# Plachtaa/FAcodec

Measured on NVIDIA H100. Metric: audio_seconds_per_second, higher is better.
Workload: dtype f32 I/O and accumulation; every product is a 3-MMA split of fp32 operands: fp16 hi + 2^11-scaled fp16 lo (22 mantissa bits, register-promoted accumulation) upstream of the VQ, bf16 hi + bf16 lo (16 bits) downstream

## Files before the change

facodec_b200/csrc/conv_tc.cu:

```cuda
#include <cuda_bf16.h>
#include <cuda_fp16.h>

#include <cstring>
#include <mutex>
#include <type_traits>

#include "common.cuh"
#include "conv_tc_common.cuh"
#include "kernels.h"

namespace fac {

namespace {

using namespace tc;

enum Prec { P_TF32 = 0, P_BF16 = 1, P_F16S = 2, P_F16X2 = 3, P_NONE = -1 };

template <int P> struct PrecT {
    static constexpr int KG = P == P_TF32 ? 4 : 2;
    static constexpr int planes = P == P_F16S ? 1 : 2;
    static constexpr int ksteps = P == P_TF32 ? 2 : 1;
    static constexpr int kind = P == P_TF32 ? WG_TF32 : (P == P_BF16 ? WG_BF16 : WG_F16);
};
// ... 28 lines not shown
#pragma unroll
    for (int j = 0; j < NI / 8; ++j) {
        if (j > 0 && (8 * j) % GROUP == 0 && 8 * j >= tl.nw) break;
#pragma unroll
        for (int h = 0; h < 2; ++h) {
            const int row = tl.row0 + 16 * tl.warp + (tl.lane >> 2) + 8 * h;
            const int col = tl.col0 + 8 * j + 2 * (tl.lane & 3);
            f(row, col, acc[4 * j + 2 * h], acc[4 * j + 2 * h + 1]);
        }
    }
}

template <bool FAST>
__device__ __forceinline__ float act_out(int act, float v, float al, float ia) {
    if (act == ACT_SNAKE) return FAST ? fmaf(ia, sin2_mufu(al * v), v) : snake_fast(v, al, ia);
    if (act == ACT_TANH) return tanhf(v);
    if (act == ACT_MISH) return mish_f(v);
    return v;
}

template <int P1, int P2, bool TT>
constexpr bool groupable() { return P1 != P_F16S && P2 == P_NONE && !TT; }

template <int P1, int P2, bool PROMO, int NI, int MINB = 1, bool TT = false>
__global__ void __launch_bounds__(kThreads, groupable<P1, P2, TT>() && NI <= 128 ? 2 : MINB) conv_tc_kernel(TcConvParams p) {
    constexpr bool FUSED = P2 != P_NONE;
    constexpr bool GROUPABLE = groupable<P1, P2, TT>();
    static_assert(!TT || (NI == 64 && !FUSED), "transposed tiles: <= 64 channels x 64 time steps per warpgroup");
    static_assert(NI % 16 == 0 && NI <= (PROMO || MINB == 2 ? 64 : (P1 == P_F16S ? 256 : 128)),
                  "accumulator registers: <= 64 / 128 columns (256 in the one-pass fp16 class at one CTA per SM)");
    constexpr bool F16X2 = P1 == P_F16X2;
    constexpr bool DEC = P1 == P_BF16 || P1 == P_F16S;
    using T1 = PrecT<P1>;
    extern __shared__ __align__(1024) uint8_t smem[];
    uint64_t* full = reinterpret_cast<uint64_t*>(smem);

    const int tid = threadIdx.x, wg = tid >> 7;
    const int BM = 64 * p.MT;
    const int N = p.N, NW = p.MT == 2 ? N : N / 2;
    Tile tl;
    tl.row0 = p.MT == 2 ? 64 * wg : 0;
    tl.col0 = p.MT == 2 ? 0 : wg * NW;
    tl.nw = NW;
    tl.warp = (tid >> 5) & 3;
    tl.lane = tid & 31;
    const int t0 = blockIdx.x * BM, ntile = blockIdx.y, b = blockIdx.z;
    const int Kr = p.Kr, dil = p.dil, Rpad = p.Rpad, nchunk = p.nchunk, S = p.stagesB;
    const int G = GROUPABLE ? p.group : 1;
    const int R = BM + (Kr - 1) * dil;
    const int nstep1 = G == 4 ? nchunk >> 2 : (G == 2 ? nchunk >> 1 : nchunk);
    const uint32_t a_plane = (uint32_t)G * T1::KG * Rpad * 16, a_bytes = a_plane * T1::planes;
    uint8_t* abuf = smem + kSmemHdr;
    float4* master = reinterpret_cast<float4*>(abuf + 2 * (size_t)a_bytes);
    uint8_t* wbuf = abuf + 2 * (size_t)a_bytes + master_bytes(PROMO, nchunk, p.promote_every, NI);
    uint8_t* a2buf = wbuf + (size_t)S * p.b_slot;
    const uint32_t w_unit1 = (uint32_t)Kr * T1::planes * T1::KG * N * 16;
    const uint32_t w_unit2 = FUSED ? (uint32_t)prec_planes(P2) * prec_kg(P2) * N * 16 : 0;
    const int units = nstep1 + (FUSED ? p.nchunk2 : 0);

    if (tid == 0) {
        for (int i = 0; i < S; ++i) mbar_init(&full[i], 1);
        fence_mbar_init();
    }
    __syncthreads();
    auto issue_w = [&](int u) {
        uint64_t* bar = &full[u % S];
        uint8_t* dst = wbuf + (size_t)(u % S) * p.b_slot;
        const uint8_t* src;
        uint32_t bytes;
        if (u < nstep1) {
            src = reinterpret_cast<const uint8_t*>(p.wblob) + ((size_t)ntile * nchunk + (size_t)u * G) * w_unit1;
            bytes = G * w_unit1;
        } else { src = reinterpret_cast<const uint8_t*>(p.wblob2) + (size_t)(u - nstep1) * w_unit2; bytes = w_unit2; }
        mbar_arrive_expect_tx(bar, bytes);
        bulk_g2s(dst, src, bytes, bar);
    };
    if (tid == 0)
        for (int u = 0; u < S - 1 && u < units; ++u) issue_w(u);

    const PadMap pm = PadMap::lane(p.lane_len, b, p.Tin, p.pad_left_s, p.pad_right_s, p.reflect);
    const float* __restrict__ xb = p.x + (size_t)b * p.x_bstride;
    auto produce = [&](int s) {
        uint8_t* ahi = abuf + (size_t)(s & 1) * a_bytes;
        auto run = [&](auto grouped) {
            constexpr bool GR = decltype(grouped)::value;
            const int c = GR ? s * G : s;
            if constexpr (P1 == P_TF32) produce_chunk<kThreads, GR, false>(p, pm, xb, c, G, t0, R, Rpad, ahi, ahi + a_plane, tid);
            else if constexpr (P1 == P_BF16) produce_chunk<kThreads, GR, true>(p, pm, xb, c, G, t0, R, Rpad, ahi, ahi + a_plane, tid);
            else if constexpr (P1 == P_F16S) produce_chunk<kThreads, GR, true, 4, false, false, true>(p, pm, xb, c, G, t0, R, Rpad, ahi, ahi, tid);
            else produce_chunk<kThreads, GR, false, 4, false, true>(p, pm, xb, c, G, t0, R, Rpad, ahi, ahi + a_plane, tid);
        };
        if constexpr (GROUPABLE) {
            if (G > 1) run(std::true_type());
            else run(std::false_type());
        } else {
            run(std::false_type());
        }
        fence_proxy_async();
    };
    produce(0);

    float acc[NI / 2];
    float crs[F16X2 ? NI / 2 : 1];
    zero_acc<NI>(acc);
    if constexpr (F16X2) zero_acc<NI>(crs);
    const uint32_t a_lbo = (uint32_t)Rpad * 16, b_lbo = (uint32_t)N * 16;
    const uint32_t abase = smem_u32(abuf), wbase = smem_u32(wbuf), a2base = smem_u32(a2buf);
    const int BM2 = BM;
// ... 20 lines not shown
        }
    };

#pragma unroll 1
    for (int u = 0; u < units; ++u) {
        __syncthreads();
        if (tid == 0 && u + S - 1 < units) issue_w(u + S - 1);
        mbar_wait(&full[u % S], (uint32_t)(u / S) & 1u);
        const uint32_t wslot = wbase + (uint32_t)(u % S) * p.b_slot;
        wg_fence();
        if (u < nstep1) {
            const uint32_t a0 = abase + (uint32_t)(u & 1) * a_bytes + (uint32_t)tl.row0 * 16;
            const uint32_t b0 = wslot + (uint32_t)tl.col0 * 16;
            auto mma_tap = [&](uint32_t ahi, uint32_t bhi) {
                const uint32_t alo = ahi + a_plane, blo = bhi + T1::KG * b_lbo;
                if constexpr (TT) {
                    mma_pass<P1, NI>(acc, bhi, b_lbo, ahi, a_lbo);
                    mma_pass<P1, NI>(crs, bhi, b_lbo, alo, a_lbo);
                    mma_pass<P1, NI>(crs, blo, b_lbo, ahi, a_lbo);
                } else if constexpr (P1 == P_F16S) {
                    mma_pass<P1, NI>(acc, ahi, a_lbo, bhi, b_lbo);
                } else if constexpr (F16X2) {
                    mma_pass<P1, NI>(acc, ahi, a_lbo, bhi, b_lbo);
                    mma_pass<P1, NI>(crs, ahi, a_lbo, blo, b_lbo);
                    mma_pass<P1, NI>(crs, alo, a_lbo, bhi, b_lbo);
                } else {
                    mma_pass<P1, NI>(acc, ahi, a_lbo, bhi, b_lbo);
                    mma_pass<P1, NI>(acc, ahi, a_lbo, blo, b_lbo);
                    mma_pass<P1, NI>(acc, alo, a_lbo, bhi, b_lbo);
                }
            };
            if constexpr (GROUPABLE) {
                uint32_t ac = a0, bc = b0, ahi = a0, bhi = b0;
#pragma unroll 1
                for (int i = 0, tap = 0; i < G * Kr; ++i) {
                    mma_tap(ahi, bhi);
                    if (++tap < Kr) { ahi += (uint32_t)dil * 16; bhi += T1::planes * T1::KG * b_lbo; }
                    else { tap = 0; ac += T1::KG * a_lbo; bc += w_unit1; ahi = ac; bhi = bc; }
                }
            } else {
#pragma unroll 1
                for (int tap = 0; tap < Kr; ++tap)
                    mma_tap(a0 + (uint32_t)(tap * dil) * 16, b0 + (uint32_t)tap * T1::planes * T1::KG * b_lbo);
            }
            wg_commit();
            if (u + 1 < nstep1) produce(u + 1);
            wg_wait_all();
            const int done = (u + 1) * G;
            if (PROMO && (done % p.promote_every == 0 || done == nchunk)) promote(done <= p.promote_every, done == nchunk);
            if constexpr (FUSED) {
                if (u + 1 == nstep1) {
                    constexpr int KG2 = prec_kg(P2 < 0 ? 0 : P2);
                    const uint32_t a2_plane = (uint32_t)(p.nchunk2 * KG2) * BM2 * 16;
                    for_each_pair<NI, 32>(tl, acc, [&](int row, int col, float v0, float v1) {
                        const float2 bi = __ldg(reinterpret_cast<const float2*>(p.bias + col));
                        const float2 al = __ldg(reinterpret_cast<const float2*>(p.out_alpha + col));
                        const float2 ia = __ldg(reinterpret_cast<const float2*>(p.out_inv_alpha + col));
                        v0 = act_out<DEC>(ACT_SNAKE, v0 + bi.x, al.x, ia.x);
                        v1 = act_out<DEC>(ACT_SNAKE, v1 + bi.y, al.y, ia.y);
                        if constexpr (P2 == P_BF16) {
                            __nv_bfloat162 h = __floats2bfloat162_rn(v0, v1);
                            float2 hf = __bfloat1622float2(h);
                            __nv_bfloat162 l = __floats2bfloat162_rn(v0 - hf.x, v1 - hf.y);
                            const uint32_t off = ((uint32_t)(col >> 3) * BM2 + row) * 16 + (col & 7) * 2;
                            *reinterpret_cast<__nv_bfloat162*>(a2buf + off) = h;
                            *reinterpret_cast<__nv_bfloat162*>(a2buf + a2_plane + off) = l;
                        } else {
                            const float h0 = to_tf32(v0), h1 = to_tf32(v1);
                            const uint32_t off = ((uint32_t)(col >> 2) * BM2 + row) * 16 + (col & 3) * 4;
                            *reinterpret_cast<float2*>(a2buf + off) = make_float2(h0, h1);
                            *reinterpret_cast<float2*>(a2buf + a2_plane + off) = make_float2(to_tf32(v0 - h0), to_tf32(v1 - h1));
                        }
                    });
                    fence_proxy_async();
                    zero_acc<NI>(acc);
                }
            }
        } else if constexpr (FUSED) {
            constexpr int P2x = P2 < 0 ? 0 : P2;
            constexpr int KG2 = prec_kg(P2x);
            const int c2 = u - nstep1;
            const uint32_t a2_plane = (uint32_t)(p.nchunk2 * KG2) * BM2 * 16, a2_lbo = (uint32_t)BM2 * 16;
            const uint32_t ahi = a2base + ((uint32_t)(c2 * KG2) * BM2 + tl.row0) * 16, alo = ahi + a2_plane;
            const uint32_t bhi = wslot + (uint32_t)tl.col0 * 16, blo = bhi + KG2 * b_lbo;
            mma_pass<P2x, NI>(acc, ahi, a2_lbo, bhi, b_lbo);
            mma_pass<P2x, NI>(acc, ahi, a2_lbo, blo, b_lbo);
            mma_pass<P2x, NI>(acc, alo, a2_lbo, bhi, b_lbo);
            wg_commit();
            wg_wait_all();
        }
    }

    const float* __restrict__ bias = FUSED ? p.bias2 : p.bias;
    const int act = FUSED ? ACT_NONE : p.out_act;
    float* __restrict__ yb = p.y + (size_t)b * p.y_bstride + (size_t)ntile * N;
    const float* __restrict__ rb = p.res ? p.res + (size_t)b * p.y_bstride + (size_t)ntile * N : nullptr;
    const float* al_p = act == ACT_SNAKE ? p.out_alpha + (size_t)ntile * N : nullptr;
    const float* ia_p = act == ACT_SNAKE ? p.out_inv_alpha + (size_t)ntile * N : nullptr;
    const float* bi_p = bias ? bias + (size_t)ntile * N : nullptr;
    if constexpr (TT) {
        for_each_pair<NI>(tl, acc, [&](int r, int c, float v0, float v1) {
            if (r - tl.row0 >= NW) return;
            const int co = tl.col0 + (r - tl.row0), tf = tl.row0 + (c - tl.col0);
            const float bi = bi_p ? __ldg(bi_p + co) : 0.f;
            const float al = act == ACT_SNAKE ? __ldg(al_p + co) : 0.f, ia = act == ACT_SNAKE ? __ldg(ia_p + co) : 0.f;
            const float v[2] = {v0, v1};
#pragma unroll
            for (int e = 0; e < 2; ++e) {
                const int t = t0 + tf + e;
                if (t >= p.Tout) continue;
                float o = act_out<DEC>(act, v[e] + bi, al, ia);
                if (rb) o += rb[(size_t)t * p.ldy + co];
                yb[(size_t)t * p.ldy + co] = o;
            }
        });
        return;
    }
    for_each_pair<NI>(tl, acc, [&](int row, int col, float v0, float v1) {
        const int t = t0 + row;
        if (t >= p.Tout) return;
        if (bi_p) { const float2 bi = __ldg(reinterpret_cast<const float2*>(bi_p + col)); v0 += bi.x; v1 += bi.y; }
        if (act == ACT_SNAKE) {
            const float2 al = __ldg(reinterpret_cast<const float2*>(al_p + col));
            const float2 ia = __ldg(reinterpret_cast<const float2*>(ia_p + col));
            v0 = act_out<DEC>(ACT_SNAKE, v0, al.x, ia.x);
            v1 = act_out<DEC>(ACT_SNAKE, v1, al.y, ia.y);
        } else if (act != ACT_NONE) {
            v0 = act_out<DEC>(act, v0, 0.f, 0.f);
            v1 = act_out<DEC>(act, v1, 0.f, 0.f);
        }
        if (rb) { const float2 r = *reinterpret_cast<const float2*>(rb + (size_t)t * p.ldy + col); v0 += r.x; v1 += r.y; }
        *reinterpret_cast<float2*>(yb + (size_t)t * p.ldy + col) = make_float2(v0, v1);
    });
}

}

namespace {
constexpr size_t kSmemCap = 227 * 1024;
constexpr size_t kSmemCap2 = 113 * 1024;
int plan_prec(const TcConvParams& p) {
    return p.g1f16 ? P_F16S : (p.f16x2 ? P_F16X2 : (p.bf16 ? P_BF16 : P_TF32));
}
constexpr int f16s_wide_nw(bool fused) { return fused ? 192 : 256; }
}

bool tc_conv_plan(TcConvParams& p) {
    if ((p.Cin % 4) != 0 || ((p.Cin * p.vf) % kChunk) != 0 || (p.Cout % 16) != 0) return false;
    if (p.bf16 && p.promoted) return false;
    if (p.f16x2 && !p.promoted) return false;
    if (p.g1f16 && !p.bf16) return false;
    if (p.tt && !p.f16x2) return false;
    if (p.fused && (p.promoted || p.Cin != p.Cout || p.vf != 1 || p.Cout > 256)) return false;
    const int P1 = plan_prec(p), P2 = p.fused ? (p.bf16 ? P_BF16 : P_TF32) : P_NONE;
    p.nchunk = p.Cin * p.vf / kChunk;
    p.nchunk2 = p.fused ? p.Cout / kChunk : 0;
    p.promote_every = p.promoted ? (p.f16x2 ? (48 / p.Kr < 1 ? 1 : 48 / p.Kr) : (8 / p.Kr < 1 ? 1 : 8 / p.Kr)) : 1;
    const int nw_max = p.promoted ? 64 : 128;
    constexpr size_t kAReserve = 40 * 1024;
    int N = 0;
    for (int cand = p.fused ? p.Cout : 256; cand >= 16 && N == 0; cand -= 16) {
        const bool rows_split = cand <= nw_max, cols_split = (cand / 2) % 16 == 0 && cand / 2 <= nw_max;
        if (p.Cout % cand || !(rows_split || cols_split)) continue;
        size_t slot = (size_t)p.Kr * prec_planes(P1) * prec_kg(P1) * cand * 16, a2 = 0;
        if (P2 != P_NONE) a2 = (size_t)prec_planes(P2) * p.nchunk2 * prec_kg(P2) * 64 * 16;
        if (kSmemHdr + kAReserve + slot + a2 <= kSmemCap) N = cand;
        else if (p.fused) return false;
    }
    if (N == 0) return false;
    struct Layout { int Rpad; size_t slot, total; };
    auto layout = [&](int S, int MT, int G) {
        const int NW = MT == 2 ? N : N / 2, BM = 64 * MT;
        Layout l;
        const int v = G == 1 ? 2 : (P1 == P_TF32 ? 1 : 4 / G);
        l.Rpad = BM + (p.Kr - 1) * p.dil;
        while (l.Rpad % 8 != v) ++l.Rpad;
        const size_t a_bytes = (size_t)G * prec_planes(P1) * prec_kg(P1) * l.Rpad * 16;
        l.slot = (size_t)G * p.Kr * prec_planes(P1) * prec_kg(P1) * N * 16;
        size_t a2 = 0;
        if (P2 != P_NONE) {
            const size_t slot2 = (size_t)prec_planes(P2) * prec_kg(P2) * N * 16;
            if (slot2 > l.slot) l.slot = slot2;
            a2 = (size_t)prec_planes(P2) * p.nchunk2 * prec_kg(P2) * BM * 16;
        }
        const size_t master = master_bytes(p.promoted, p.nchunk, p.promote_every, p.tt ? 64 : NW);
        l.total = kSmemHdr + 2 * a_bytes + master + S * l.slot + a2 + (p.tt ? 64 * 16 : 0);
        return l;
    };
    auto group = [&](int S, int MT, size_t cap) {
        if (p.Kr > 3 || p.tt || p.fused || p.g1f16) return 1;
        for (int G = 4; G > 1; G /= 2)
            if (G <= p.max_group && p.nchunk % G == 0 && (!p.promoted || p.promote_every % G == 0) && layout(S, MT, G).total <= cap) return G;
        return 1;
    };
    const bool want2 = p.promoted ? !p.tt : (p.occ2_maxn > 0 && N <= p.occ2_maxn);
    for (int two = want2 ? 1 : 0; two >= 0; --two) {
        const size_t cap = two ? kSmemCap2 : kSmemCap;
        const int nwl = two ? 64 : nw_max;
        for (int S = 2; S >= 1; --S)
            for (int MT = 2; MT >= 1; --MT) {
                const int NW = MT == 2 ? N : N / 2;
                const bool wide = !two && P1 == P_F16S && NW == f16s_wide_nw(p.fused);
                if ((NW > nwl && !wide) || NW % 16) continue;
                if (wide && layout(2, 1, 1).total <= kSmemCap2) continue;
                const Layout l1 = layout(S, MT, 1);
                if (l1.total > cap) continue;
                const int G = group(S, MT, l1.total <= kSmemCap2 ? kSmemCap2 : cap);
                const Layout l = layout(S, MT, G);
                p.N = N; p.MT = MT; p.Rpad = l.Rpad; p.R2pad = 64 * MT; p.stagesB = S; p.b_slot = (int)l.slot;
                p.group = G;
                p.smem_bytes = l.total;
                p.occ2 = two;
                return true;
            }
    }
    return false;
}

size_t tc_blob_floats(const TcConvParams& p) {
    if (p.g1f16) return (size_t)(p.Cout / p.N) * p.nchunk * p.Kr * 2 * p.N * 4;
    return (size_t)(p.Cout / p.N) * p.nchunk * p.Kr * 2 * ((p.bf16 || p.f16x2) ? 2 : 4) * p.N * 4;
}

static inline uint16_t bf16_rn_host(float f) {
    uint32_t u;
    memcpy(&u, &f, 4);
    u += 0x7FFFu + ((u >> 16) & 1u);
    return (uint16_t)(u >> 16);
}

void tc_pack_blob(const TcConvParams& p, const float* wp, int ldw, float* blob) {
    const int Cw = p.Cin * p.vf;
    if (p.g1f16) {
        uint16_t* ob = reinterpret_cast<uint16_t*>(blob);
        size_t o16 = 0;
        for (int nt = 0; nt < p.Cout / p.N; ++nt)
            for (int c = 0; c < p.nchunk; ++c)
                for (int tap = 0; tap < p.Kr; ++tap)
                    for (int k8 = 0; k8 < 2; ++k8)
                        for (int n = 0; n < p.N; ++n)
                            for (int e = 0; e < 8; ++e) {
                                int kk = tap * Cw + c * tc::kChunk + k8 * 8 + e;
                                __half v = __float2half_rn(wp[(size_t)kk * ldw + nt * p.N + n]);
                                uint16_t bits;
                                memcpy(&bits, &v, 2);
                                ob[o16++] = bits;
                            }
        return;
    }
    if (p.f16x2) {
        uint16_t* ob = reinterpret_cast<uint16_t*>(blob);
        size_t o16 = 0;
        for (int nt = 0; nt < p.Cout / p.N; ++nt)
            for (int c = 0; c < p.nchunk; ++c)
                for (int tap = 0; tap < p.Kr; ++tap)
                    for (int hl = 0; hl < 2; ++hl)
// ... 51 lines not shown
                                lu = (lu + 0x1000u) & 0xFFFFE000u;
                                float lo_r;
                                memcpy(&lo_r, &lu, 4);
                                blob[o++] = hl == 0 ? hi : lo_r;
                            }
}

namespace {
template <int P1, int P2, bool PROMO, int NI, int MINB = 1, bool TT = false>
cudaError_t launch_one(const TcConvParams& p, dim3 grid, cudaStream_t st) {
    static bool done[64] = {};
    static std::mutex mu;
    int dev = 0;
    cudaError_t e = cudaGetDevice(&dev);
    if (e != cudaSuccess) return e;
    if (dev < 0 || dev >= 64) return cudaErrorInvalidDevice;
    {
        std::lock_guard<std::mutex> lk(mu);
        if (!done[dev]) {
            e = cudaFuncSetAttribute(conv_tc_kernel<P1, P2, PROMO, NI, MINB, TT>, cudaFuncAttributeMaxDynamicSharedMemorySize,
                                     (int)kSmemCap);
            if (e != cudaSuccess) return e;
            done[dev] = true;
        }
    }
    conv_tc_kernel<P1, P2, PROMO, NI, MINB, TT><<<grid, kThreads, p.smem_bytes, st>>>(p);
    return cudaGetLastError();
}
template <int P1, int P2, bool PROMO, int MINB = 1, int NI = (PROMO || MINB == 2 ? 64 : 128)>
cudaError_t launch_nw(const TcConvParams& p, dim3 grid, cudaStream_t st) {
    const int NW = p.MT == 2 ? p.N : p.N / 2;
    if (NW == NI) return launch_one<P1, P2, PROMO, NI, MINB>(p, grid, st);
    if constexpr (NI > 16) return launch_nw<P1, P2, PROMO, MINB, NI - 16>(p, grid, st);
    else return cudaErrorInvalidValue;
}
template <int P1, int P2>
cudaError_t launch_occ(const TcConvParams& p, dim3 grid, cudaStream_t st) {
    if (p.occ2) return launch_nw<P1, P2, false, 2>(p, grid, st);
    if constexpr (P1 == P_F16S) {
        constexpr int kWide = f16s_wide_nw(P2 != P_NONE);
        if ((p.MT == 2 ? p.N : p.N / 2) == kWide) return launch_one<P1, P2, false, kWide>(p, grid, st);
    }
    return launch_nw<P1, P2, false, 1>(p, grid, st);
}
}

cudaError_t launch_conv_tc(const TcConvParams& p, cudaStream_t st) {
    if (p.Tout <= 0 || p.B <= 0) return cudaSuccess;
    const int BM = 64 * p.MT;
    dim3 grid((p.Tout + BM - 1) / BM, p.Cout / p.N, p.B);
    if (grid.y > 65535 || grid.z > 65535) return cudaErrorInvalidValue;
    const int P1 = plan_prec(p);
    if (p.fused) {
        if (P1 == P_F16S) return launch_occ<P_F16S, P_BF16>(p, grid, st);
        if (P1 == P_BF16) return launch_occ<P_BF16, P_BF16>(p, grid, st);
        return launch_occ<P_TF32, P_TF32>(p, grid, st);
    }
    if (p.tt) return launch_one<P_F16X2, P_NONE, true, 64, 1, true>(p, grid, st);
    if (p.promoted)
        return P1 == P_F16X2 ? launch_nw<P_F16X2, P_NONE, true, 2>(p, grid, st) : launch_nw<P_TF32, P_NONE, true, 2>(p, grid, st);
    if (P1 == P_F16S) return launch_occ<P_F16S, P_NONE>(p, grid, st);
    if (P1 == P_BF16) return launch_occ<P_BF16, P_NONE>(p, grid, st);
    return launch_occ<P_TF32, P_NONE>(p, grid, st);
}

}
```

facodec_b200/csrc/engine.cu:

```cuda
#include <cmath>
#include <cstdio>
#include <cstdlib>
#include <cstring>
#include <algorithm>
#include <initializer_list>
#include <map>
#include <memory>
#include <string>
#include <type_traits>
#include <vector>

#include "../../include/facodec_b200.h"
#include "../../include/facodec_b200_debug.h"
#include "common.cuh"
#include "kernels.h"

using namespace fac;

namespace {

constexpr int HOP = 300;
constexpr int LATENT = 1024;
constexpr int N_FFT = 2048;
constexpr int WIN = 1200;
// ... 656 lines not shown
            tp.B = B; tp.Tin = Tin; tp.ldx = w.Cin;
            tp.PLr = o.pad_left / w.vf;
            tp.pad_left_s = o.pad_left; tp.pad_right_s = o.pad_right; tp.reflect = o.reflect; tp.lane_len = o.lane_len;
            tp.Tout = Tout; tp.ldy = w.Cout;
            tp.x_bstride = (size_t)Tin * w.Cin; tp.y_bstride = (size_t)Tout * w.Cout;
            double flops = 2.0 * B * Tout * (double)w.Cout * w.K * w.Cin;
            double bytes = 4.0 * ((double)B * Tin * w.Cin + (double)B * Tout * w.Cout * (o.res ? 2 : 1) + (double)w.K * w.Cin * w.Cout);
            char det[96];
            snprintf(det, sizeof det, "%s Cin%d Cout%d K%d d%d T%d", name, w.Cin, w.Cout, w.K, o.dil, Tout);
            c.begin(tp.promoted ? "conv_tcp" : "conv_tc", flops, bytes, det);
            c.check(launch_conv_tc(tp, c.st), name);
            c.end();
            return;
        }
    }
    ConvParams p;
    p.x = x; p.y = y;
    p.w = c.W(w.w);
    p.bias = o.no_bias ? nullptr : c.W(w.b);
    if (o.in_snake) { p.in_alpha = c.W(o.in_snake->a); p.in_inv_alpha = c.W(o.in_snake->ia); }
    p.out_act = o.act;
    if (o.out_snake) { p.out_act = ACT_SNAKE; p.out_alpha = c.W(o.out_snake->a); p.out_inv_alpha = c.W(o.out_snake->ia); }
    p.res = o.res; p.valid_len = o.valid_len; p.lane_len = o.lane_len;
    p.B = B; p.Tin = Tin; p.Cin = w.Cin; p.Tout = Tout; p.Cout = w.Cout;
    p.K = w.K; p.dil = o.dil; p.stride = o.stride;
    p.pad_left = o.pad_left; p.pad_right = o.pad_right; p.pad_reflect = o.reflect;
    p.ldw = w.ldw; p.ldy = o.ldy ? o.ldy : w.Cout; p.ldx = o.ldx ? o.ldx : w.Cin;
    p.y_transposed = o.transposed;
    p.x_bstride = (size_t)Tin * p.ldx;
    p.y_bstride = (size_t)Tout * p.ldy;
    double flops = 2.0 * B * Tout * (double)w.Cout * w.K * w.Cin;
    double bytes = 4.0 * ((double)B * Tin * w.Cin + (double)B * Tout * w.Cout * (o.res ? 2 : 1) + (double)w.K * w.Cin * w.Cout);
    char det[96];
    snprintf(det, sizeof det, "%s Cin%d Cout%d K%d d%d T%d", name, w.Cin, w.Cout, w.K, o.dil, Tout);
    c.begin("conv", flops, bytes, det);
    c.check(launch_conv(p, c.st), name);
    c.end();
}

int sconv(Ctx& c, const ConvW& w, const float* x, float* y, int B, int T, int dil, int stride, ConvOpts o,
          const char* name, bool causal = true) {
    int k_eff = (w.K - 1) * dil + 1;
    o.dil = dil; o.stride = stride;
    const int total = k_eff - stride, extra = conv_extra_pad(T, k_eff, stride);
    o.pad_left = causal ? total : total - total / 2;
    o.pad_right = (causal ? 0 : total / 2) + extra;
    o.reflect = 1;
    int Tout = conv_out_len(T, k_eff, stride);
    run_conv(c, w, x, y, B, T, Tout, o, name);
    return Tout;
}

bool residual_unit_fused(Ctx& c, const ResW& r, const float* x, float* y, int B, int T, bool causal, const int* lane_len) {
    if (c.h->use_tc < 1 || !c.h->fuse_res || c.vq_critical || !r.c7.tc || !r.c1.tc || r.c7.promoted || r.c1.promoted ||
        r.c7.Cin != r.c7.Cout || r.c1.K != 1 || r.c7.vf != 1)
        return false;
    TcConvParams tp;
    tp.Cin = r.c7.Cin; tp.Cout = r.c7.Cout; tp.vf = 1; tp.Kr = r.c7.K; tp.dil = r.dil; tp.fused = 1;
    tp.bf16 = (c.h->dec_bf16 && r.c7.has16 && r.c1.has16) ? 1 : 0;
    tp.g1f16 = (tp.bf16 && r.c7.has_f16s && c.h->dec_c7_f16) ? 1 : 0;
    tp.occ2_maxn = c.h->tc_occ2;
    tp.Tout = T;
    if (c.h->fuse_res == 2 && r.c7.Cout > 128) return false;
    if (!tc_conv_plan(tp)) return false;
    TcConvParams q7 = tp, q1 = tp;
    q7.fused = 0; q1.fused = 0; q1.Kr = 1; q1.g1f16 = 0;
    if (!tc_conv_plan(q7) || !tc_conv_plan(q1) || q7.N != tp.N || q1.N != tp.N) return false;
    if (c.dry) return true;
    const int k_eff = (r.c7.K - 1) * r.dil + 1;
    tp.x = x; tp.y = y; tp.res = x;
    tp.wblob = c.W(tp.g1f16 ? r.c7.tcw_f16s : (tp.bf16 ? r.c7.tcw16 : r.c7.tcw)); tp.bias = c.W(r.c7.b);
    tp.wblob2 = c.W(tp.bf16 ? r.c1.tcw16 : r.c1.tcw); tp.bias2 = c.W(r.c1.b);
    tp.in_alpha = c.W(r.s1.a); tp.in_inv_alpha = c.W(r.s1.ia);
    tp.out_act = ACT_SNAKE; tp.out_alpha = c.W(r.s2.a); tp.out_inv_alpha = c.W(r.s2.ia);
    tp.B = B; tp.Tin = T; tp.ldx = r.c7.Cin;
    const int pl = causal ? k_eff - 1 : (k_eff - 1) - (k_eff - 1) / 2;
    tp.PLr = pl; tp.pad_left_s = pl; tp.pad_right_s = k_eff - 1 - pl; tp.reflect = 1; tp.lane_len = lane_len;
    tp.Tout = T; tp.ldy = r.c7.Cout;
    tp.x_bstride = (size_t)T * r.c7.Cin; tp.y_bstride = (size_t)T * r.c7.Cout;
    double flops = 2.0 * B * T * (double)r.c7.Cout * r.c7.Cin * (r.c7.K + 1);
    double bytes = 4.0 * ((double)B * T * r.c7.Cin * 2 + (double)B * T * r.c7.Cout + (double)(r.c7.K + 1) * r.c7.Cin * r.c7.Cout);
    char det[96];
    snprintf(det, sizeof det, "res.fused C%d K%d d%d T%d", r.c7.Cin, r.c7.K, r.dil, T);
    c.begin("conv_tc", flops, bytes, det);
    c.check(launch_conv_tc(tp, c.st), "res.fused");
    c.end();
    return true;
}

void residual_unit(Ctx& c, const ResW& r, const float* x, float* tmp, float* y, int B, int T, bool causal = true,
                   const int* lane_len = nullptr) {
    if (residual_unit_fused(c, r, x, y, B, T, causal, lane_len)) return;
    ConvOpts o1;
    o1.in_snake = &r.s1;
    o1.out_snake = &r.s2;
    o1.lane_len = lane_len;
    sconv(c, r.c7, x, tmp, B, T, r.dil, 1, o1, "res.conv7", causal);
    ConvOpts o2;
    o2.res = x;
    sconv(c, r.c1, tmp, y, B, T, 1, 1, o2, "res.conv1", causal);
}

int lstm_pass3(const Ctx& c) { return (c.vq_critical || !c.h->dec_bf16) ? 1 : 0; }
bool lstm_resident(const Ctx& c, const LstmW& L) {
    const int pass3 = lstm_pass3(c);
    return c.h->lstm_v2 && L.has2[pass3] && (pass3 || c.h->dec_lstm_fp16);
}

void slstm(Ctx& c, const LstmW& L, const float* x, float* y, int B, int T, LstmState* st = nullptr, const int* lens = nullptr) {
    const int H = L.H;
    float* xg = c.alloc<float>((size_t)B * T * 4 * H);
    float* h1 = c.alloc<float>((size_t)B * T * H);
    float* hT = c.alloc<float>((size_t)2 * H * 32);
    uint32_t* h16 = c.alloc<uint32_t>((size_t)2 * 2 * (H / 2) * 32);
    unsigned int* bar = c.alloc<unsigned int>(64);
    for (int l = 0; l < 2; ++l) {
        const float* in = l == 0 ? x : h1;
        ConvOpts o;
        run_conv(c, L.ih[l], in, xg, 1, B * T, B * T, o, "lstm.ih");
        if (c.dry) continue;
        const int pass3 = lstm_pass3(c);
        const bool v2 = lstm_resident(c, L);
        for (int b0 = 0; b0 < B; b0 += 32) {
            int nb = B - b0 < 32 ? B - b0 : 32;
            LstmParams p;
            p.xg = xg + (size_t)b0 * T * 4 * H;
            p.whh_p = c.W(L.whh[l]);
            if (c.h->dec_bf16 && L.has16 && !c.vq_critical) { p.bf16 = 1; p.whh_p16 = c.W(L.whh16[l]); }
            p.skip = l == 1 ? x + (size_t)b0 * T * H : nullptr;
            p.y = (l == 0 ? h1 : y) + (size_t)b0 * T * H;
            p.hT = hT; p.bar = bar;
            p.B = nb; p.T = T; p.H = H; p.U = L.U; p.G = L.G;
            c.begin("lstm_rec", 2.0 * nb * T * 4.0 * H * H, 4.0 * ((double)nb * T * 5 * H + 4.0 * H * H));
            if ((st || lens) && (!v2 || B > 32 || !st)) {
                c.check(cudaErrorNotSupported, "lstm.stream (needs the resident-W kernel and B <= 32)"); c.end(); continue;
            }
            if (v2) {
// ... 2846 lines not shown
    return FAC_OK;
}

int fac_debug_conv_tc(fac_handle* h, const float* x, const float* w_host, const float* bias_host, int B, int Tin, int Cin,
                      int Cout, int K, int dil, int stride, int pad_left, int pad_right, int reflect,
                      const float* in_alpha_host, const float* out_alpha_host, int act, const float* res, float* y,
                      int Tout, int promoted, void* stream) {
    return debug_conv_tc(h, x, w_host, bias_host, B, Tin, Cin, Cout, K, dil, stride, pad_left, pad_right, reflect,
                         in_alpha_host, out_alpha_host, act, res, y, Tout, promoted, stream, nullptr, nullptr);
}

int fac_debug_conv_tc_group1(fac_handle* h, const float* x, const float* w_host, const float* bias_host, int B, int Tin,
                             int Cin, int Cout, int K, int dil, int stride, int pad_left, int pad_right, int reflect,
                             const float* in_alpha_host, const float* out_alpha_host, int act, const float* res, float* y,
                             int Tout, int promoted, void* stream, int* group) {
    if (!group) return FAC_ERR_INVALID;
    return debug_conv_tc(h, x, w_host, bias_host, B, Tin, Cin, Cout, K, dil, stride, pad_left, pad_right, reflect,
                         in_alpha_host, out_alpha_host, act, res, y, Tout, promoted, stream, group, nullptr);
}

int fac_debug_conv_lanes(fac_handle* h, const float* x, const float* w_host, const float* bias_host, int B, int Tin,
                         int Cin, int Cout, int K, int dil, int stride, int pad_left, int pad_right, int reflect,
                         const float* in_alpha_host, const float* out_alpha_host, int act, const float* res, float* y,
                         int Tout, int path, const int* lane_len_host, void* stream) {
    if (!h || !x || !w_host || !y || B <= 0 || Tin <= 0) return FAC_ERR_INVALID;
    int* lanes = nullptr;
    int rc = debug_upload_lanes(h, "fac_debug_conv_lanes", lane_len_host, B, Tin, &lanes);
    if (rc != FAC_OK) return rc;
    if (path == -1)
        rc = debug_conv(h, x, w_host, bias_host, B, Tin, Cin, Cout, K, dil, stride, pad_left, pad_right, reflect,
                        in_alpha_host, out_alpha_host, act, res, y, Tout, lanes, stream);
    else
        rc = debug_conv_tc(h, x, w_host, bias_host, B, Tin, Cin, Cout, K, dil, stride, pad_left, pad_right, reflect,
                           in_alpha_host, out_alpha_host, act, res, y, Tout, path, stream, nullptr, lanes);
    cudaFree(lanes);
    return rc;
}

int fac_debug_resunit(fac_handle* h, const float* x, const float* w7_host, const float* b7_host, const float* w1_host,
                      const float* b1_host, const float* alpha1_host, const float* alpha2_host, int B, int T, int C,
                      int dil, int mode, float* y, void* stream) {
    return fac_debug_resunit_lanes(h, x, w7_host, b7_host, w1_host, b1_host, alpha1_host, alpha2_host, B, T, C, dil, mode,
                                   1, nullptr, y, stream);
}

int fac_debug_resunit_lanes(fac_handle* h, const float* x, const float* w7_host, const float* b7_host,
                            const float* w1_host, const float* b1_host, const float* alpha1_host,
                            const float* alpha2_host, int B, int T, int C, int dil, int mode, int causal,
                            const int* lane_len_host, float* y, void* stream) {
    if (!h || !x || !y || !w7_host || !w1_host || B <= 0 || T <= 0) return FAC_ERR_INVALID;
    int* lanes = nullptr;
    int rc0 = debug_upload_lanes(h, "fac_debug_resunit_lanes", lane_len_host, B, T, &lanes);
    if (rc0 != FAC_OK) return rc0;
    fac_handle tmp;
    tmp.device = h->device;
    tmp.use_tc = mode == 0 ? 0 : 1;
    tmp.fuse_res = (mode == 2 || mode == 4 || mode == 6) ? 1 : 0;
    tmp.dec_bf16 = mode >= 3;
    tmp.dec_c7_f16 = mode >= 5;
    tmp.tc_occ2 = h->tc_occ2;
    auto put = [&](const char* key, const float* d, std::vector<int64_t> shp) {
        HostTensor t;
        t.shape = shp;
        t.data.assign(d, d + t.numel());
        tmp.host[0][key] = std::move(t);
    };
    put("u.block.0.alpha", alpha1_host, {1, C, 1});
    put("u.block.1.conv.conv.weight", w7_host, {C, C, 7});
    put("u.block.1.conv.conv.bias", b7_host, {C});
    put("u.block.2.alpha", alpha2_host, {1, C, 1});
    put("u.block.3.conv.conv.weight", w1_host, {C, C, 1});
    put("u.block.3.conv.conv.bias", b1_host, {C});
    ResW r;
    try { r = pack_res(&tmp, 0, "u", dil, false); } catch (const PackError& e) { h->err = e.msg; cudaFree(lanes); return FAC_ERR_STATE; }
    cudaSetDevice(h->device);
    cudaError_t e = cudaMalloc(&tmp.warena, (tmp.pack.size() + 64) * sizeof(float));
    if (e == cudaSuccess) e = cudaMemcpy(tmp.warena, tmp.pack.data(), tmp.pack.size() * sizeof(float), cudaMemcpyHostToDevice);
    if (e != cudaSuccess) { h->err = cudaGetErrorString(e); cudaGetLastError(); cudaFree(lanes); return FAC_ERR_CUDA; }
    cudaStream_t st = (cudaStream_t)stream;
    float* scratch = nullptr;
    e = cudaMalloc(&scratch, sizeof(float) * (size_t)B * T * C);
    int rc = FAC_OK;
    if (e != cudaSuccess) { h->err = cudaGetErrorString(e); rc = FAC_ERR_CUDA; }
    if (rc == FAC_OK) {
        Ctx c{&tmp, st, false};
        residual_unit(c, r, x, scratch, y, B, T, causal != 0, lanes);
        rc = finish(&tmp, c);
        cudaError_t e2 = cudaStreamSynchronize(st);
        if (rc == FAC_OK && e2 != cudaSuccess) { tmp.err = cudaGetErrorString(e2); rc = FAC_ERR_CUDA; }
        if (rc == FAC_OK && (mode == 2 || mode == 4 || mode == 6) && tmp.launches != 1) { tmp.err = "fused path not taken for this geometry"; rc = FAC_ERR_UNSUPPORTED; }
    }
    if (rc != FAC_OK) h->err = tmp.err;
    if (scratch) cudaFree(scratch);
    cudaFree(tmp.warena);
    cudaFree(lanes);
    return rc;
}

long long fac_debug_lstm_pack(const float* whh_host, int H, int bf16, float* out, long long capacity_floats, int* info3) {
    if (!whh_host || H <= 0) return FAC_ERR_INVALID;
    fac_handle tmp;
    const char* names[8] = {"weight_ih_l0", "weight_hh_l0", "bias_ih_l0", "bias_hh_l0", "weight_ih_l1", "weight_hh_l1", "bias_ih_l1", "bias_hh_l1"};
    for (int i = 0; i < 8; ++i) {
        HostTensor t;
        const bool mat = (i % 4) < 2;
        if (mat) t.shape = {4 * H, H}; else t.shape = {4 * H};
        if (i == 1) t.data.assign(whh_host, whh_host + (size_t)4 * H * H);
        else t.data.assign(t.numel(), 0.f);
        tmp.host[0][std::string("l.") + names[i]] = std::move(t);
    }
    LstmW L;
    try { L = pack_lstm(&tmp, 0, "l"); } catch (const PackError&) { return FAC_ERR_UNSUPPORTED; }
    if (info3) { info3[0] = L.U; info3[1] = L.G; info3[2] = 4 * L.U; }
    if (bf16 == 2 || bf16 == 3) {
        const int p3 = bf16 == 3;
        const long long n2 = (long long)lstm2_pack_words(H, L.U, p3);
        if (!out || capacity_floats < n2) return n2;
        lstm2_pack(whh_host, H, L.U, p3, reinterpret_cast<uint32_t*>(out));
        return n2;
    }
    const long long n = (long long)L.G * H * 4 * L.U;
    if (bf16 && !L.has16) return FAC_ERR_UNSUPPORTED;
    if (!out || capacity_floats < n) return n;
    memcpy(out, tmp.pack.data() + (bf16 ? L.whh16[0] : L.whh[0]), sizeof(float) * (size_t)n);
    return n;
}

long long fac_debug_convtr_pack(const float* w_host, int Cin, int Cout, int stride, int causal, float* out, long long capacity_floats) {
    if (!w_host || Cin <= 0 || Cout <= 0 || stride <= 0) return FAC_ERR_INVALID;
    fac_handle tmp;
    HostTensor t, b;
    t.shape = {Cin, Cout, 2 * stride};
    t.data.assign(w_host, w_host + (size_t)Cin * Cout * 2 * stride);
    b.shape = {Cout};
    b.data.assign(Cout, 0.f);
    tmp.host[0]["c.weight"] = std::move(t);
    tmp.host[0]["c.bias"] = std::move(b);
    ConvW c;
    try { c = causal ? pack_convtr(&tmp, 0, "c", stride) : pack_convtr_noncausal(&tmp, 0, "c", stride); }
    catch (const PackError&) { return FAC_ERR_UNSUPPORTED; }
    const long long n = (long long)c.K * Cin * c.Cout;
    if (!out || capacity_floats < n) return n;
    for (int k = 0; k < c.K; ++k)
        for (int ci = 0; ci < Cin; ++ci)
            for (int co = 0; co < c.Cout; ++co) out[((size_t)k * Cin + ci) * c.Cout + co] = tmp.pack[c.w + ((size_t)k * Cin + ci) * c.ldw + co];
    return n;
}

int fac_debug_pad_map(int L, int pad_left, int pad_right, int reflect, int* out, int n) {
    if (!out || L < 0 || pad_left < 0 || pad_right < 0 || n != pad_left + L + pad_right) return FAC_ERR_INVALID;
    const PadMap pm = PadMap::make(L, pad_left, pad_right, reflect);
    for (int i = 0; i < n; ++i) out[i] = pm.src(i - pad_left);
    return FAC_OK;
}

int fac_debug_lane_pad_map(const int* lane_len, int B, int Tin, int pad_left, int pad_right, int reflect, int* out, int n) {
    if (!out || B <= 0 || Tin < 0 || pad_left < 0 || pad_right < 0 || n != pad_left + Tin + pad_right) return FAC_ERR_INVALID;
    for (int b = 0; lane_len && b < B; ++b)
        if (lane_len[b] < 0 || lane_len[b] > Tin) return FAC_ERR_INVALID;
    for (int b = 0; b < B; ++b) {
        const PadMap pm = PadMap::lane(lane_len, b, Tin, pad_left, pad_right, reflect);
        for (int i = 0; i < n; ++i) out[(size_t)b * n + i] = pm.src(i - pad_left);
    }
    return FAC_OK;
}

static int debug_tc_plan(int Cin, int Cout, int K, int dil, int stride, int Tout, int mode, int occ2_maxn, TcConvParams& tp) {
    if (Cin <= 0 || Cout <= 0 || K <= 0 || dil <= 0 || stride <= 0 || mode < 0 || mode > 8) return FAC_ERR_INVALID;
    tp.Cin = Cin; tp.Cout = Cout; tp.Tout = Tout; tp.occ2_maxn = occ2_maxn;
    tp.promoted = (mode == 1 || mode == 3) ? 1 : 0;
    tp.bf16 = (mode == 2 || mode == 4 || mode == 7 || mode == 8) ? 1 : 0;
    tp.f16x2 = mode == 3 ? 1 : 0;
    tp.fused = (mode == 4 || mode == 5 || mode == 8) ? 1 : 0;
    tp.g1f16 = (mode == 7 || mode == 8) ? 1 : 0;
    if (mode == 6) { tp.promoted = 1; tp.f16x2 = 1; tp.tt = 1; }
    if (stride == 1) { tp.vf = 1; tp.Kr = K; tp.dil = dil; }
    else if (K == 2 * stride && dil == 1) { tp.vf = stride; tp.Kr = 2; tp.dil = 1; }
    else return FAC_ERR_UNSUPPORTED;
    return tc_conv_plan(tp) ? FAC_OK : FAC_ERR_UNSUPPORTED;
}

int fac_debug_tc_plan(int Cin, int Cout, int K, int dil, int stride, int Tout, int mode, int occ2_maxn, int* out8) {
    if (!out8) return FAC_ERR_INVALID;
    TcConvParams tp;
    const int rc = debug_tc_plan(Cin, Cout, K, dil, stride, Tout, mode, occ2_maxn, tp);
    if (rc != FAC_OK) return rc;
    out8[0] = tp.N; out8[1] = tp.MT; out8[2] = tp.nchunk; out8[3] = tp.stagesB; out8[4] = tp.R2pad;
    out8[5] = (int)tp.smem_bytes; out8[6] = tp.Rpad; out8[7] = tp.promote_every;
    return FAC_OK;
}

int fac_debug_tc_plan_group(int Cin, int Cout, int K, int dil, int stride, int Tout, int mode, int occ2_maxn, int* smem2) {
    TcConvParams tp;
    const int rc = debug_tc_plan(Cin, Cout, K, dil, stride, Tout, mode, occ2_maxn, tp);
    if (rc != FAC_OK) return rc;
    if (smem2) {
        TcConvParams t1 = tp;
        t1.max_group = 1;
        if (!tc_conv_plan(t1)) return FAC_ERR_UNSUPPORTED;
        smem2[0] = (int)tp.smem_bytes;
        smem2[1] = (int)t1.smem_bytes;
    }
    return tp.group;
}

long long fac_debug_tc_pack(const float* w_host, int Cin, int Cout, int K, int stride, int mode, float* blob_out,
                            long long capacity_floats) {
    if (!w_host || Cin <= 0 || Cout <= 0 || K <= 0 || stride <= 0 || mode < 0 || mode > 3) return FAC_ERR_INVALID;
    TcConvParams tp;
    tp.Cin = Cin; tp.Cout = Cout; tp.dil = 1;
    tp.promoted = (mode == 1 || mode == 3) ? 1 : 0; tp.bf16 = mode == 2 ? 1 : 0; tp.f16x2 = mode == 3 ? 1 : 0;
    if (stride == 1) { tp.vf = 1; tp.Kr = K; }
    else if (K == 2 * stride) { tp.vf = stride; tp.Kr = 2; }
    else return FAC_ERR_UNSUPPORTED;
    if (!tc_conv_plan(tp)) return FAC_ERR_UNSUPPORTED;
    const long long n = (long long)tc_blob_floats(tp);
    if (!blob_out || capacity_floats < n) return n;
    const int ldw = (Cout + 3) / 4 * 4;
    std::vector<float> gen((size_t)K * Cin * ldw, 0.f);
    for (int co = 0; co < Cout; ++co)
        for (int ci = 0; ci < Cin; ++ci)
            for (int k = 0; k < K; ++k) gen[((size_t)k * Cin + ci) * ldw + co] = w_host[((size_t)co * Cin + ci) * K + k];
    tc_pack_blob(tp, gen.data(), ldw, blob_out);
    return n;
}

// ... 101 lines not shown
```

Baseline: 1015.

## Fuse promoted fp16x2 residual-unit convolutions on the encoder (pre-VQ) path

Extends the fused residual-unit kernel (k-tap conv, snake activation, then 1x1 conv) to the promoted fp16 hi/lo precision mode, so encoder residual units upstream of the VQ can run as a single launch instead of two. The intermediate activation is split into fp16 hi plus a scaled fp16 lo and staged in shared memory that reuses the promotion master buffer, with an added block barrier. The second stage accumulates its cross terms into a separate register accumulator and promotes at the end. The intent is to cut the extra launch and the global-memory round trip of the intermediate. The cost is tighter planner constraints (NW=64, two-CTA occupancy, N==Cout) and aliasing of shared buffers.

```diff
diff --git a/facodec_b200/csrc/conv_tc.cu b/facodec_b200/csrc/conv_tc.cu
--- a/facodec_b200/csrc/conv_tc.cu
+++ b/facodec_b200/csrc/conv_tc.cu
@@ -104,8 +104,9 @@
     const uint32_t a_plane = (uint32_t)G * T1::KG * Rpad * 16, a_bytes = a_plane * T1::planes;
     uint8_t* abuf = smem + kSmemHdr;
     float4* master = reinterpret_cast<float4*>(abuf + 2 * (size_t)a_bytes);
-    uint8_t* wbuf = abuf + 2 * (size_t)a_bytes + master_bytes(PROMO, nchunk, p.promote_every, NI);
-    uint8_t* a2buf = wbuf + (size_t)S * p.b_slot;
+    const uint32_t m_bytes = master_bytes(PROMO, nchunk, p.promote_every, NI);
+    uint8_t* wbuf = abuf + 2 * (size_t)a_bytes + m_bytes;
+    uint8_t* a2buf = m_bytes ? reinterpret_cast<uint8_t*>(master) : wbuf + (size_t)S * p.b_slot;
     const uint32_t w_unit1 = (uint32_t)Kr * T1::planes * T1::KG * N * 16;
     const uint32_t w_unit2 = FUSED ? (uint32_t)prec_planes(P2) * prec_kg(P2) * N * 16 : 0;
     const int units = nstep1 + (FUSED ? p.nchunk2 : 0);
@@ -232,6 +233,7 @@
                 if (u + 1 == nstep1) {
                     constexpr int KG2 = prec_kg(P2 < 0 ? 0 : P2);
                     const uint32_t a2_plane = (uint32_t)(p.nchunk2 * KG2) * BM2 * 16;
+                    if (m_bytes) __syncthreads();
                     for_each_pair<NI, 32>(tl, acc, [&](int row, int col, float v0, float v1) {
                         const float2 bi = __ldg(reinterpret_cast<const float2*>(p.bias + col));
                         const float2 al = __ldg(reinterpret_cast<const float2*>(p.out_alpha + col));
@@ -245,6 +247,13 @@
                             const uint32_t off = ((uint32_t)(col >> 3) * BM2 + row) * 16 + (col & 7) * 2;
                             *reinterpret_cast<__nv_bfloat162*>(a2buf + off) = h;
                             *reinterpret_cast<__nv_bfloat162*>(a2buf + a2_plane + off) = l;
+                        } else if constexpr (P2 == P_F16X2) {
+                            const __half2 h = __floats2half2_rn(v0, v1);
+                            const float2 hf = __half22float2(h);
+                            const __half2 l = __floats2half2_rn((v0 - hf.x) * kLoScale, (v1 - hf.y) * kLoScale);
+                            const uint32_t off = ((uint32_t)(col >> 3) * BM2 + row) * 16 + (col & 7) * 2;
+                            *reinterpret_cast<__half2*>(a2buf + off) = h;
+                            *reinterpret_cast<__half2*>(a2buf + a2_plane + off) = l;
                         } else {
                             const float h0 = to_tf32(v0), h1 = to_tf32(v1);
                             const uint32_t off = ((uint32_t)(col >> 2) * BM2 + row) * 16 + (col & 3) * 4;
@@ -263,11 +272,18 @@
             const uint32_t a2_plane = (uint32_t)(p.nchunk2 * KG2) * BM2 * 16, a2_lbo = (uint32_t)BM2 * 16;
             const uint32_t ahi = a2base + ((uint32_t)(c2 * KG2) * BM2 + tl.row0) * 16, alo = ahi + a2_plane;
             const uint32_t bhi = wslot + (uint32_t)tl.col0 * 16, blo = bhi + KG2 * b_lbo;
-            mma_pass<P2x, NI>(acc, ahi, a2_lbo, bhi, b_lbo);
-            mma_pass<P2x, NI>(acc, ahi, a2_lbo, blo, b_lbo);
-            mma_pass<P2x, NI>(acc, alo, a2_lbo, bhi, b_lbo);
+            if constexpr (P2x == P_F16X2) {
+                mma_pass<P2x, NI>(acc, ahi, a2_lbo, bhi, b_lbo);
+                mma_pass<P2x, NI>(crs, ahi, a2_lbo, blo, b_lbo);
+                mma_pass<P2x, NI>(crs, alo, a2_lbo, bhi, b_lbo);
+            } else {
+                mma_pass<P2x, NI>(acc, ahi, a2_lbo, bhi, b_lbo);
+                mma_pass<P2x, NI>(acc, ahi, a2_lbo, blo, b_lbo);
+                mma_pass<P2x, NI>(acc, alo, a2_lbo, bhi, b_lbo);
+            }
             wg_commit();
             wg_wait_all();
+            if (PROMO && c2 + 1 == p.nchunk2) promote(true, true);
         }
     }
 
@@ -331,11 +347,12 @@
     if (p.f16x2 && !p.promoted) return false;
     if (p.g1f16 && !p.bf16) return false;
     if (p.tt && !p.f16x2) return false;
-    if (p.fused && (p.promoted || p.Cin != p.Cout || p.vf != 1 || p.Cout > 256)) return false;
-    const int P1 = plan_prec(p), P2 = p.fused ? (p.bf16 ? P_BF16 : P_TF32) : P_NONE;
+    if (p.fused && ((p.promoted && (!p.f16x2 || p.tt)) || p.Cin != p.Cout || p.vf != 1 || p.Cout > 256)) return false;
+    const int P1 = plan_prec(p), P2 = p.fused ? (p.f16x2 ? P_F16X2 : (p.bf16 ? P_BF16 : P_TF32)) : P_NONE;
     p.nchunk = p.Cin * p.vf / kChunk;
     p.nchunk2 = p.fused ? p.Cout / kChunk : 0;
     p.promote_every = p.promoted ? (p.f16x2 ? (48 / p.Kr < 1 ? 1 : 48 / p.Kr) : (8 / p.Kr < 1 ? 1 : 8 / p.Kr)) : 1;
+    if (p.fused && p.promoted && p.nchunk2 > 48) return false;
     const int nw_max = p.promoted ? 64 : 128;
     constexpr size_t kAReserve = 40 * 1024;
     int N = 0;
@@ -347,7 +364,7 @@
         if (kSmemHdr + kAReserve + slot + a2 <= kSmemCap) N = cand;
         else if (p.fused) return false;
     }
-    if (N == 0) return false;
+    if (N == 0 || (p.fused && p.promoted && N != p.Cout)) return false;
     struct Layout { int Rpad; size_t slot, total; };
     auto layout = [&](int S, int MT, int G) {
         const int NW = MT == 2 ? N : N / 2, BM = 64 * MT;
@@ -364,6 +381,7 @@
             a2 = (size_t)prec_planes(P2) * p.nchunk2 * prec_kg(P2) * BM * 16;
         }
         const size_t master = master_bytes(p.promoted, p.nchunk, p.promote_every, p.tt ? 64 : NW);
+        if (master) a2 = 0;
         l.total = kSmemHdr + 2 * a_bytes + master + S * l.slot + a2 + (p.tt ? 64 * 16 : 0);
         return l;
     };
@@ -373,15 +391,16 @@
             if (G <= p.max_group && p.nchunk % G == 0 && (!p.promoted || p.promote_every % G == 0) && layout(S, MT, G).total <= cap) return G;
         return 1;
     };
+    const bool unit2 = p.fused && p.promoted;
     const bool want2 = p.promoted ? !p.tt : (p.occ2_maxn > 0 && N <= p.occ2_maxn);
-    for (int two = want2 ? 1 : 0; two >= 0; --two) {
+    for (int two = want2 ? 1 : 0; two >= (unit2 ? 1 : 0); --two) {
         const size_t cap = two ? kSmemCap2 : kSmemCap;
         const int nwl = two ? 64 : nw_max;
         for (int S = 2; S >= 1; --S)
             for (int MT = 2; MT >= 1; --MT) {
                 const int NW = MT == 2 ? N : N / 2;
                 const bool wide = !two && P1 == P_F16S && NW == f16s_wide_nw(p.fused);
-                if ((NW > nwl && !wide) || NW % 16) continue;
+                if ((NW > nwl && !wide) || NW % 16 || (unit2 && NW != 64)) continue;
                 if (wide && layout(2, 1, 1).total <= kSmemCap2) continue;
                 const Layout l1 = layout(S, MT, 1);
                 if (l1.total > cap) continue;
@@ -539,6 +558,8 @@
     if (grid.y > 65535 || grid.z > 65535) return cudaErrorInvalidValue;
     const int P1 = plan_prec(p);
     if (p.fused) {
+        if (P1 == P_F16X2)
+            return (p.MT == 2 ? p.N : p.N / 2) == 64 ? launch_one<P_F16X2, P_F16X2, true, 64, 2>(p, grid, st) : cudaErrorInvalidValue;
         if (P1 == P_F16S) return launch_occ<P_F16S, P_BF16>(p, grid, st);
         if (P1 == P_BF16) return launch_occ<P_BF16, P_BF16>(p, grid, st);
         return launch_occ<P_TF32, P_TF32>(p, grid, st);
diff --git a/facodec_b200/csrc/engine.cu b/facodec_b200/csrc/engine.cu
--- a/facodec_b200/csrc/engine.cu
+++ b/facodec_b200/csrc/engine.cu
@@ -732,12 +732,18 @@
 }
 
 bool residual_unit_fused(Ctx& c, const ResW& r, const float* x, float* y, int B, int T, bool causal, const int* lane_len) {
-    if (c.h->use_tc < 1 || !c.h->fuse_res || c.vq_critical || !r.c7.tc || !r.c1.tc || r.c7.promoted || r.c1.promoted ||
-        r.c7.Cin != r.c7.Cout || r.c1.K != 1 || r.c7.vf != 1)
+    const bool promoted = r.c7.promoted && r.c1.promoted;
+    if (!c.h->fuse_res || !r.c7.tc || !r.c1.tc || r.c7.promoted != r.c1.promoted || r.c7.Cin != r.c7.Cout ||
+        r.c1.K != 1 || r.c7.vf != 1)
+        return false;
+    if (c.vq_critical ? (!promoted || c.h->use_tc < 2 || !c.h->enc_f16 || c.h->enc_tt || !r.c7.has16 || !r.c1.has16)
+                      : (promoted || c.h->use_tc < 1))
         return false;
     TcConvParams tp;
     tp.Cin = r.c7.Cin; tp.Cout = r.c7.Cout; tp.vf = 1; tp.Kr = r.c7.K; tp.dil = r.dil; tp.fused = 1;
-    tp.bf16 = (c.h->dec_bf16 && r.c7.has16 && r.c1.has16) ? 1 : 0;
+    tp.promoted = promoted ? 1 : 0;
+    tp.f16x2 = tp.promoted;
+    tp.bf16 = (!promoted && c.h->dec_bf16 && r.c7.has16 && r.c1.has16) ? 1 : 0;
     tp.g1f16 = (tp.bf16 && r.c7.has_f16s && c.h->dec_c7_f16) ? 1 : 0;
     tp.occ2_maxn = c.h->tc_occ2;
     tp.Tout = T;
@@ -749,8 +755,8 @@
     if (c.dry) return true;
     const int k_eff = (r.c7.K - 1) * r.dil + 1;
     tp.x = x; tp.y = y; tp.res = x;
-    tp.wblob = c.W(tp.g1f16 ? r.c7.tcw_f16s : (tp.bf16 ? r.c7.tcw16 : r.c7.tcw)); tp.bias = c.W(r.c7.b);
-    tp.wblob2 = c.W(tp.bf16 ? r.c1.tcw16 : r.c1.tcw); tp.bias2 = c.W(r.c1.b);
+    tp.wblob = c.W(tp.g1f16 ? r.c7.tcw_f16s : ((tp.bf16 || tp.f16x2) ? r.c7.tcw16 : r.c7.tcw)); tp.bias = c.W(r.c7.b);
+    tp.wblob2 = c.W((tp.bf16 || tp.f16x2) ? r.c1.tcw16 : r.c1.tcw); tp.bias2 = c.W(r.c1.b);
     tp.in_alpha = c.W(r.s1.a); tp.in_inv_alpha = c.W(r.s1.ia);
     tp.out_act = ACT_SNAKE; tp.out_alpha = c.W(r.s2.a); tp.out_inv_alpha = c.W(r.s2.ia);
     tp.B = B; tp.Tin = T; tp.ldx = r.c7.Cin;
@@ -762,7 +768,7 @@
     double bytes = 4.0 * ((double)B * T * r.c7.Cin * 2 + (double)B * T * r.c7.Cout + (double)(r.c7.K + 1) * r.c7.Cin * r.c7.Cout);
     char det[96];
     snprintf(det, sizeof det, "res.fused C%d K%d d%d T%d", r.c7.Cin, r.c7.K, r.dil, T);
-    c.begin("conv_tc", flops, bytes, det);
+    c.begin(tp.promoted ? "conv_tcp" : "conv_tc", flops, bytes, det);
     c.check(launch_conv_tc(tp, c.st), "res.fused");
     c.end();
     return true;
@@ -3715,12 +3721,14 @@
     int* lanes = nullptr;
     int rc0 = debug_upload_lanes(h, "fac_debug_resunit_lanes", lane_len_host, B, T, &lanes);
     if (rc0 != FAC_OK) return rc0;
+    if (mode < 0 || mode > 8) { cudaFree(lanes); return FAC_ERR_INVALID; }
     fac_handle tmp;
     tmp.device = h->device;
-    tmp.use_tc = mode == 0 ? 0 : 1;
-    tmp.fuse_res = (mode == 2 || mode == 4 || mode == 6) ? 1 : 0;
-    tmp.dec_bf16 = mode >= 3;
-    tmp.dec_c7_f16 = mode >= 5;
+    const bool enc = mode >= 7, fused = mode == 2 || mode == 4 || mode == 6 || mode == 8;
+    tmp.use_tc = mode == 0 ? 0 : (enc ? 2 : 1);
+    tmp.fuse_res = fused ? 1 : 0;
+    tmp.dec_bf16 = mode >= 3 && !enc;
+    tmp.dec_c7_f16 = mode >= 5 && !enc;
     tmp.tc_occ2 = h->tc_occ2;
     auto put = [&](const char* key, const float* d, std::vector<int64_t> shp) {
         HostTensor t;
@@ -3735,7 +3743,7 @@
     put("u.block.3.conv.conv.weight", w1_host, {C, C, 1});
     put("u.block.3.conv.conv.bias", b1_host, {C});
     ResW r;
-    try { r = pack_res(&tmp, 0, "u", dil, false); } catch (const PackError& e) { h->err = e.msg; cudaFree(lanes); return FAC_ERR_STATE; }
+    try { r = pack_res(&tmp, 0, "u", dil, enc); } catch (const PackError& e) { h->err = e.msg; cudaFree(lanes); return FAC_ERR_STATE; }
     cudaSetDevice(h->device);
     cudaError_t e = cudaMalloc(&tmp.warena, (tmp.pack.size() + 64) * sizeof(float));
     if (e == cudaSuccess) e = cudaMemcpy(tmp.warena, tmp.pack.data(), tmp.pack.size() * sizeof(float), cudaMemcpyHostToDevice);
@@ -3747,11 +3755,12 @@
     if (e != cudaSuccess) { h->err = cudaGetErrorString(e); rc = FAC_ERR_CUDA; }
     if (rc == FAC_OK) {
         Ctx c{&tmp, st, false};
+        c.vq_critical = enc;
         residual_unit(c, r, x, scratch, y, B, T, causal != 0, lanes);
         rc = finish(&tmp, c);
         cudaError_t e2 = cudaStreamSynchronize(st);
         if (rc == FAC_OK && e2 != cudaSuccess) { tmp.err = cudaGetErrorString(e2); rc = FAC_ERR_CUDA; }
-        if (rc == FAC_OK && (mode == 2 || mode == 4 || mode == 6) && tmp.launches != 1) { tmp.err = "fused path not taken for this geometry"; rc = FAC_ERR_UNSUPPORTED; }
+        if (rc == FAC_OK && fused && tmp.launches != 1) { tmp.err = "fused path not taken for this geometry"; rc = FAC_ERR_UNSUPPORTED; }
     }
     if (rc != FAC_OK) h->err = tmp.err;
     if (scratch) cudaFree(scratch);
@@ -3829,12 +3838,12 @@
 }
 
 static int debug_tc_plan(int Cin, int Cout, int K, int dil, int stride, int Tout, int mode, int occ2_maxn, TcConvParams& tp) {
-    if (Cin <= 0 || Cout <= 0 || K <= 0 || dil <= 0 || stride <= 0 || mode < 0 || mode > 8) return FAC_ERR_INVALID;
+    if (Cin <= 0 || Cout <= 0 || K <= 0 || dil <= 0 || stride <= 0 || mode < 0 || mode > 9) return FAC_ERR_INVALID;
     tp.Cin = Cin; tp.Cout = Cout; tp.Tout = Tout; tp.occ2_maxn = occ2_maxn;
-    tp.promoted = (mode == 1 || mode == 3) ? 1 : 0;
+    tp.promoted = (mode == 1 || mode == 3 || mode == 9) ? 1 : 0;
     tp.bf16 = (mode == 2 || mode == 4 || mode == 7 || mode == 8) ? 1 : 0;
-    tp.f16x2 = mode == 3 ? 1 : 0;
-    tp.fused = (mode == 4 || mode == 5 || mode == 8) ? 1 : 0;
+    tp.f16x2 = (mode == 3 || mode == 9) ? 1 : 0;
+    tp.fused = (mode == 4 || mode == 5 || mode == 8 || mode == 9) ? 1 : 0;
     tp.g1f16 = (mode == 7 || mode == 8) ? 1 : 0;
     if (mode == 6) { tp.promoted = 1; tp.f16x2 = 1; tp.tt = 1; }
     if (stride == 1) { tp.vf = 1; tp.Kr = K; tp.dil = dil; }
```

Result: faster. 1063 (median of 6 runs) (+4.8%).
